# vsois/hanabi-agents

Measured on AMD Instinct MI355X. Metric: env_steps_per_sec, higher is better.
Workload: dtype u8 env/encoder + bfloat16 Q-net GEMM (fp32 accumulate, fp32 master weights)

## Files before the change

### hanabi-agents_amd/csrc/actor_fused.hip

```cpp
#include <hip/hip_runtime.h>
#include <hip/hip_bf16.h>
#include <hip/hip_fp16.h>

#include <cstdint>
#include <type_traits>

#include "../../include/hanabi_hip.h"
#include "common.hpp"
#include "env_kernel.hpp"

using hb::fail;

namespace {

typedef __bf16 bf16x8 __attribute__((ext_vector_type(8)));
typedef _Float16 f16x8 __attribute__((ext_vector_type(8)));
typedef float f32x4 __attribute__((ext_vector_type(4)));

constexpr int FM = 128;
constexpr int FH = 512;
constexpr int FNT = 512;
constexpr int FK = 51;
constexpr int S2 = FH / 32;
constexpr int LUT_BYTES = 65536;
constexpr int H_BYTES = FM * FH * 2;
constexpr int FRAG_FLOATS = 3 * 8 * FM;
constexpr int LDS_TOTAL = H_BYTES + FRAG_FLOATS * 4;
constexpr float NEG_BIG = -1e30f;

struct FusedArgs {
  const uint32_t* obs;
  long long m;
  int words;
  int s1;
  const uint4* w1f;
  const float* b1;
  const uint4* w2f;
  const float* b2;
  const float* support;
  float* q;
  int n_actions, n_pass;
  const int8_t* legal;
  int32_t* actions;
  float epsilon;
  unsigned long long seed, draw;
  long long first_gid;
  unsigned long long* stamps;
};

#ifdef HB_STAMPS
#define HB_FSTAMP(slot)                                                                              \
  do {                                                                                               \
    __builtin_amdgcn_sched_barrier(0);                                                               \
    unsigned long long hb_t_;                                                                        \
    asm volatile("s_memtime %0\n\ts_waitcnt lgkmcnt(0)" : "=s"(hb_t_)::"memory");                    \
    if (a.stamps && lane == 0) a.stamps[(static_cast<long long>(blockIdx.x) * 8 + wave) * 16 + (slot)] = hb_t_; \
    __builtin_amdgcn_sched_barrier(0);                                                               \
  } while (0)
#define HB_FSTAMP_REAL(slot)                                                                         \
  do {                                                                                               \
    unsigned long long hb_t_;                                                                        \
    asm volatile("s_memrealtime %0\n\ts_waitcnt lgkmcnt(0)" : "=s"(hb_t_)::"memory");                \
    if (a.stamps && lane == 0) a.stamps[(static_cast<long long>(blockIdx.x) * 8 + wave) * 16 + (slot)] = hb_t_; \
  } while (0)
#else
#define HB_FSTAMP(slot) do {} while (0)
#define HB_FSTAMP_REAL(slot) do {} while (0)
#endif

template <bool F16>
__device__ __forceinline__ uint32_t pack16(float lo, float hi) {
  if constexpr (F16) {
    const _Float16 a = static_cast<_Float16>(lo), b = static_cast<_Float16>(hi);
    uint16_t ua, ub;
    __builtin_memcpy(&ua, &a, 2);
    __builtin_memcpy(&ub, &b, 2);
    return static_cast<uint32_t>(ua) | (static_cast<uint32_t>(ub) << 16);
  } else {
    const __hip_bfloat16 a = __float2bfloat16(lo), b = __float2bfloat16(hi);
    return static_cast<uint32_t>(*reinterpret_cast<const uint16_t*>(&a)) |
           (static_cast<uint32_t>(*reinterpret_cast<const uint16_t*>(&b)) << 16);
  }
}
template <bool F16>
__device__ __forceinline__ uint32_t bits2_one(uint32_t b, int p) {
  const uint32_t t = (b >> (2 * p)) & 3u;
  return __umul24((t | (t << 15)) & 0x00010001u, F16 ? 0x3C00u : 0x3F80u);
}
template <bool F16>
__device__ __forceinline__ f32x4 mfma16(const uint4& wv, const uint4& xv, const f32x4& c) {
  if constexpr (F16) {
    union { uint4 u; f16x8 f; } w, x;
    w.u = wv; x.u = xv;
    return __builtin_amdgcn_mfma_f32_16x16x32_f16(w.f, x.f, c, 0, 0, 0);
  } else {
    union { uint4 u; bf16x8 f; } w, x;
    w.u = wv; x.u = xv;
    return __builtin_amdgcn_mfma_f32_16x16x32_bf16(w.f, x.f, c, 0, 0, 0);
  }
}
typedef float f32x2 __attribute__((ext_vector_type(2)));
typedef unsigned int u32x2 __attribute__((ext_vector_type(2)));
__device__ __forceinline__ float vmax(float a, float b) {
  float r;
  asm("v_max_f32 %0, %1, %2" : "=v"(r) : "v"(a), "v"(b));
  return r;
}
__device__ __forceinline__ float vmax3(float a, float b, float c) {
  float r;
  asm("v_max3_f32 %0, %1, %2, %3" : "=v"(r) : "v"(a), "v"(b), "v"(c));
  return r;
}
__device__ __forceinline__ float exp2_fast(float x) { return __builtin_amdgcn_exp2f(x); }

template <bool F16, class K, int EG>
__device__ __forceinline__ void actor_fused_body(const FusedArgs& a) {
  __shared__ __attribute__((aligned(16))) unsigned char lds[LDS_TOTAL];
  const int tid = threadIdx.x, lane = tid & 63;
  const int wave = __builtin_amdgcn_readfirstlane(tid >> 6);
  const int r = lane & 15, qd = lane >> 4;
  const long long row0 = static_cast<long long>(blockIdx.x) * FM;
  const int s1 = a.s1, G = (s1 + 3) >> 2;
  unsigned char* lutb = lds + (LDS_TOTAL - LUT_BYTES);
  const int bits_off = LDS_TOTAL - LUT_BYTES - 2048 * G;
  unsigned char* bits = lds + bits_off;
  const int m_early = bits_off >> 14;

  HB_FSTAMP_REAL(14);
  HB_FSTAMP(0);
  const uint4* w1p = a.w1f + (4 * wave) * 64 + lane;
  uint4 wa[4], wb[4];
#pragma unroll
  for (int n = 0; n < 4; ++n) wa[n] = w1p[n * 64];

  uint32_t w[4] = {0u, 0u, 0u, 0u};
  auto load_item = [&](int it) {
    const int rr = it & (FM - 1), g = it >> 7;
    long long row = row0 + rr;
    if (row >= a.m) row = a.m - 1;
    const uint32_t* src = a.obs + row * a.words + 4 * g;
#pragma unroll
    for (int i = 0; i < 4; ++i) w[i] = (4 * g + i < a.words) ? src[i] : 0u;
  };
  if (tid < FM * G) load_item(tid);
  for (int e = tid; e < 4096; e += FNT) {
    const uint32_t v = static_cast<uint32_t>(e) >> 4;
    *reinterpret_cast<uint4*>(lutb + e * 16) = make_uint4(bits2_one<F16>(v, 0), bits2_one<F16>(v, 1), bits2_one<F16>(v, 2), bits2_one<F16>(v, 3));
  }
  for (int it = tid; it < FM * G; it += FNT) {
    const int rr = it & (FM - 1), g = it >> 7;
    if (it != tid) load_item(it);
    uint32_t* dst = reinterpret_cast<uint32_t*>(bits) + (static_cast<size_t>((rr >> 4) * G + g) * 64 + (rr & 15));
#pragma unroll
    for (int qq = 0; qq < 4; ++qq) {
      const uint32_t o = ((w[0] >> (8 * qq)) & 0xFFu) | (((w[1] >> (8 * qq)) & 0xFFu) << 8) | (((w[2] >> (8 * qq)) & 0xFFu) << 16) |
                         (((w[3] >> (8 * qq)) & 0xFFu) << 24);
      dst[qq * 16] = o;
    }
  }
  HB_FSTAMP(1);
  __syncthreads();
  HB_FSTAMP(2);

  f32x4 acc[4][8];
#pragma unroll
  for (int n = 0; n < 4; ++n) {
    const float4 b = *reinterpret_cast<const float4*>(a.b1 + 64 * wave + 16 * n + 4 * qd);
#pragma unroll
    for (int m = 0; m < 8; ++m) acc[n][m] = f32x4{b.x, b.y, b.z, b.w};
  }

  {
    const unsigned char* lut = lutb + r * 16;
    const uint32_t* bw = reinterpret_cast<const uint32_t*>(bits) + lane;
#define HB_L1_STEP(I, WCUR, WNXT, HAVE_NEXT)                                                                   \
  {                                                                                                            \
    const int s_ = 4 * g + (I);                                                                                \
    if (HAVE_NEXT) {                                                                                           \
      _Pragma("unroll") for (int n = 0; n < 4; ++n) WNXT[n] = w1p[(s_ + 1) * 2048 + n * 64];                    \
    }                                                                                                          \
    asm volatile("" ::: "memory");                \
    uint4 xf[8];                                                                                               \
    _Pragma("unroll") for (int m = 0; m < 8; ++m) {                                                            \
      const uint32_t v = (xw[m] >> (8 * (I))) & 0xFFu;                                                         \
      xf[m] = *reinterpret_cast<const uint4*>(lut + v * 256u);                                                 \
    }                                                                                                          \
    _Pragma("unroll") for (int n = 0; n < 4; ++n) {                                                            \
      _Pragma("unroll") for (int m = 0; m < 8; ++m)                                                            \
        acc[n][m] = mfma16<F16>(WCUR[n], xf[m], acc[n][m]);                                                    \
    }                                                                                                          \
  }
    for (int g = 0; g < G; ++g) {
      uint32_t xw[8];
#pragma unroll
      for (int m = 0; m < 8; ++m) xw[m] = bw[(m * G + g) * 64];
      HB_L1_STEP(0, wa, wb, true)
      const bool more = 4 * g + 2 < s1;
      HB_L1_STEP(1, wb, wa, more)
      if (more) {
        HB_L1_STEP(2, wa, wb, true)
        HB_L1_STEP(3, wb, wa, (4 * g + 4 < s1))
      }
    }
#undef HB_L1_STEP
  }
  HB_FSTAMP(3);

  const uint4* w2p = a.w2f + (4 * wave) * 64 + lane;
#pragma unroll
  for (int n = 0; n < 4; ++n) wa[n] = w2p[n * 64];

#define HB_H_WRITE(COND)                                                                                        \
  _Pragma("unroll") for (int m = 0; m < 8; ++m) {                                                               \
    if (COND) {                                                                                                 \
      _Pragma("unroll") for (int n = 0; n < 4; ++n) {                                                           \
        const int chunk = 8 * wave + 2 * n + (qd >> 1);                                                         \
        const float v0 = fmaxf(acc[n][m][0], 0.f), v1 = fmaxf(acc[n][m][1], 0.f);                               \
        const float v2 = fmaxf(acc[n][m][2], 0.f), v3 = fmaxf(acc[n][m][3], 0.f);                               \
        *reinterpret_cast<uint2*>(lds + (16 * m + r) * 1024 + ((chunk ^ r) << 4) + (qd & 1) * 8) =              \
            make_uint2(pack16<F16>(v0, v1), pack16<F16>(v2, v3));                                               \
      }                                                                                                         \
    }                                                                                                           \
  }
  HB_H_WRITE(m < m_early)
  HB_FSTAMP(4);
  __syncthreads();
  HB_H_WRITE(m >= m_early)
#undef HB_H_WRITE

  HB_FSTAMP(5);
  __syncthreads();
  HB_FSTAMP(6);

  const int n_pass = a.n_pass, A = a.n_actions;
  const int full_cap = 8 * n_pass;
  constexpr float LOG2E = 1.44269504088896340736f;
  const unsigned char* hrow = lds + r * 1024;

  for (int p = 0; p < n_pass; ++p) {
    const int slot = 8 * p + wave;
    {
      const float* bp = a.b2 + static_cast<long long>(slot) * 64 + 4 * qd;
#pragma unroll
      for (int n = 0; n < 4; ++n) {
        const float4 b = *reinterpret_cast<const float4*>(bp + 16 * n);
#pragma unroll
        for (int m = 0; m < 8; ++m) acc[n][m] = f32x4{b.x, b.y, b.z, b.w};
      }
    }
    const uint4* wp = w2p + static_cast<long long>(p) * S2 * 2048;
#define HB_L2_HALF(S, WCUR, M0)                                                                                \
  {                                                                                                            \
    uint4 xf[4];                                                                                               \
    const int ch = ((4 * (S) + qd) ^ r) << 4;                                                                  \
    _Pragma("unroll") for (int m = 0; m < 4; ++m) xf[m] = *reinterpret_cast<const uint4*>(hrow + ((M0) + m) * 16384 + ch); \
    _Pragma("unroll") for (int n = 0; n < 4; ++n) {                                                            \
      _Pragma("unroll") for (int m = 0; m < 4; ++m)                                                            \
        acc[n][(M0) + m] = mfma16<F16>(WCUR[n], xf[m], acc[n][(M0) + m]);                                      \
    }                                                                                                          \
  }
#define HB_L2_STEP(S, WCUR, WNXT, HAVE_NEXT)                                                                   \
  {                                                                                                            \
    if (HAVE_NEXT) {                                                                                           \
      _Pragma("unroll") for (int n = 0; n < 4; ++n) WNXT[n] = wp[((S) + 1) * 2048 + n * 64];                    \
    }                                                                                                          \
    asm volatile("" ::: "memory");                                                                             \
    HB_L2_HALF(S, WCUR, 0)                                                                                     \
    __builtin_amdgcn_sched_barrier(0);                                                                         \
    HB_L2_HALF(S, WCUR, 4)                                                                                     \
  }
#pragma unroll 1
    for (int s = 0; s < S2; s += 2) {
      HB_L2_STEP(s, wa, wb, true)
      HB_L2_STEP(s + 1, wb, wa, (s + 2 < S2))
    }
#undef HB_L2_STEP
#undef HB_L2_HALF
    if (p < 2) HB_FSTAMP(7 + 3 * p);
    if (p + 1 < n_pass) {
#pragma unroll
      for (int n = 0; n < 4; ++n) wa[n] = wp[S2 * 2048 + n * 64];
    }

    auto sup_at = [&](int k) { return a.support[k < FK ? k : FK - 1]; };
    f32x2 supF[6];
#pragma unroll
    for (int i = 0; i < 6; ++i) supF[i] = f32x2{sup_at(4 * (2 * i) + qd), sup_at(4 * (2 * i + 1) + qd)};
    const float supF12 = sup_at(48 + qd);
    const int fq = wave & 3;
    const f32x2 supZa = f32x2{sup_at(13 * fq + qd), sup_at(13 * fq + 4 + qd)};
    const f32x2 supZb = f32x2{sup_at(13 * fq + 8 + qd), sup_at(13 * fq + 12)};
    const bool full_ok = slot < A && slot < full_cap;
    float* fb = reinterpret_cast<float*>(lds + H_BYTES) + wave * FM;
    const f32x2 L2 = f32x2{LOG2E, LOG2E};
    hb::static_for<2>([&](auto MH) {
    constexpr int M0 = 4 * decltype(MH)::value;
    float qF[4], zm[4], zs[4], zt[4], vf12[4], vz3[4], nmx[4], nmz[4];
#define HB_M for (int m = 0; m < 4; ++m)
#define HB_SWAP16(X, OP) { const u32x2 t_ = __builtin_amdgcn_permlane16_swap(__float_as_uint(X), __float_as_uint(X), false, false); \
                           X = OP(__uint_as_float(t_.x), __uint_as_float(t_.y)); }
#define HB_SWAP32(X, OP) { const u32x2 t_ = __builtin_amdgcn_permlane32_swap(__float_as_uint(X), __float_as_uint(X), false, false); \
                           X = OP(__uint_as_float(t_.x), __uint_as_float(t_.y)); }
#define HB_ADD(A_, B_) ((A_) + (B_))
#pragma unroll
    HB_M { vf12[m] = qd < 3 ? acc[3][M0 + m][0] : NEG_BIG; vz3[m] = qd == 3 ? acc[3][M0 + m][0] : NEG_BIG; }
#pragma unroll
    HB_M nmx[m] = vmax3(acc[0][M0 + m][0], acc[0][M0 + m][1], acc[0][M0 + m][2]);
#pragma unroll
    HB_M nmx[m] = vmax3(nmx[m], acc[0][M0 + m][3], acc[1][M0 + m][0]);
#pragma unroll
    HB_M nmx[m] = vmax3(nmx[m], acc[1][M0 + m][1], acc[1][M0 + m][2]);
#pragma unroll
    HB_M nmx[m] = vmax3(nmx[m], acc[1][M0 + m][3], acc[2][M0 + m][0]);
#pragma unroll
    HB_M nmx[m] = vmax3(nmx[m], acc[2][M0 + m][1], acc[2][M0 + m][2]);
#pragma unroll
    HB_M nmx[m] = vmax3(nmx[m], acc[2][M0 + m][3], vf12[m]);
#pragma unroll
    HB_M nmz[m] = vmax(vmax3(acc[3][M0 + m][1], acc[3][M0 + m][2], acc[3][M0 + m][3]), vz3[m]);
#pragma unroll
    HB_M HB_SWAP16(nmx[m], vmax)
#pragma unroll
    HB_M HB_SWAP16(nmz[m], vmax)
#pragma unroll
    HB_M HB_SWAP32(nmx[m], vmax)
#pragma unroll
    HB_M HB_SWAP32(nmz[m], vmax)
#pragma unroll
    HB_M { nmx[m] *= -LOG2E; nmz[m] *= -LOG2E; }
    f32x2 s2[4], t2[4];
#define HB_PAIR_FIRST(N, LO, SUP)                                                                   \
  _Pragma("unroll") HB_M {                                                                          \
    const f32x2 arg = f32x2{acc[N][M0 + m][LO], acc[N][M0 + m][LO + 1]} * L2 + f32x2{nmx[m], nmx[m]};         \
    const f32x2 e = f32x2{exp2_fast(arg.x), exp2_fast(arg.y)};                                      \
    s2[m] = e;                                                                                      \
    t2[m] = e * SUP;                                                                                \
  }
#define HB_PAIR(N, LO, SUP)                                                                         \
  _Pragma("unroll") HB_M {                                                                          \
    const f32x2 arg = f32x2{acc[N][M0 + m][LO], acc[N][M0 + m][LO + 1]} * L2 + f32x2{nmx[m], nmx[m]};         \
    const f32x2 e = f32x2{exp2_fast(arg.x), exp2_fast(arg.y)};                                      \
    s2[m] += e;                                                                                     \
    t2[m] += e * SUP;                                                                               \
  }
    HB_PAIR_FIRST(0, 0, supF[0])
    HB_PAIR(0, 2, supF[1])
    HB_PAIR(1, 0, supF[2])
    HB_PAIR(1, 2, supF[3])
    HB_PAIR(2, 0, supF[4])
    HB_PAIR(2, 2, supF[5])
#undef HB_PAIR
#undef HB_PAIR_FIRST
    float sF[4], tF[4];
#pragma unroll
    HB_M {
      const float e12 = exp2_fast(vf12[m] * LOG2E + nmx[m]);
      sF[m] = s2[m].x + s2[m].y + e12;
      tF[m] = t2[m].x + t2[m].y + e12 * supF12;
    }
#pragma unroll
    HB_M {
      const f32x2 arg = f32x2{acc[3][M0 + m][1], acc[3][M0 + m][2]} * L2 + f32x2{nmz[m], nmz[m]};
      const f32x2 e = f32x2{exp2_fast(arg.x), exp2_fast(arg.y)};
      s2[m] = e;
      t2[m] = e * supZa;
    }
#pragma unroll
    HB_M {
      const f32x2 arg = f32x2{acc[3][M0 + m][3], vz3[m]} * L2 + f32x2{nmz[m], nmz[m]};
      const f32x2 e = f32x2{exp2_fast(arg.x), exp2_fast(arg.y)};
      s2[m] += e;
      t2[m] += e * supZb;
    }
#pragma unroll
    HB_M { zs[m] = s2[m].x + s2[m].y; zt[m] = t2[m].x + t2[m].y; }
#pragma unroll
    HB_M HB_SWAP16(sF[m], HB_ADD)
#pragma unroll
    HB_M HB_SWAP16(tF[m], HB_ADD)
#pragma unroll
    HB_M HB_SWAP16(zs[m], HB_ADD)
#pragma unroll
    HB_M HB_SWAP16(zt[m], HB_ADD)
#pragma unroll
    HB_M HB_SWAP32(sF[m], HB_ADD)
#pragma unroll
    HB_M HB_SWAP32(tF[m], HB_ADD)
#pragma unroll
    HB_M HB_SWAP32(zs[m], HB_ADD)
#pragma unroll
    HB_M HB_SWAP32(zt[m], HB_ADD)
#pragma unroll
    HB_M { zm[m] = -nmz[m]; qF[m] = tF[m] * __builtin_amdgcn_rcpf(sF[m]) * (1.0f / FK); }
#undef HB_M
#undef HB_SWAP16
#undef HB_SWAP32
#undef HB_ADD
    if (qd == 0) {
#pragma unroll
      for (int m = 0; m < 4; ++m) {
        const long long row = row0 + 16 * (M0 + m) + r;
        if (full_ok && row < a.m) a.q[row * A + slot] = qF[m];
        fb[16 * (M0 + m) + r] = zm[m];
        fb[8 * FM + 16 * (M0 + m) + r] = zs[m];
        fb[16 * FM + 16 * (M0 + m) + r] = zt[m];
      }
    }
    __builtin_amdgcn_sched_barrier(0);
    });
    if (p < 2) HB_FSTAMP(8 + 3 * p);
    __syncthreads();
    if (tid < 2 * FM) {
      const int rr = tid & (FM - 1), g = tid >> 7;
      const int ea = full_cap + 2 * p + g;
      const long long row = row0 + rr;
      if (ea < A && row < a.m) {
        const float* f = reinterpret_cast<const float*>(lds + H_BYTES) + (4 * g) * FM + rr;
        const float m0 = f[0], m1 = f[FM], m2 = f[2 * FM], m3 = f[3 * FM];
        const float M = fmaxf(fmaxf(m0, m1), fmaxf(m2, m3));
        const float e0 = exp2_fast(m0 - M), e1 = exp2_fast(m1 - M), e2 = exp2_fast(m2 - M), e3 = exp2_fast(m3 - M);
        const float* fs = f + 8 * FM;
        const float* ft = f + 16 * FM;
        const float S = fs[0] * e0 + fs[FM] * e1 + fs[2 * FM] * e2 + fs[3 * FM] * e3;
        const float T = ft[0] * e0 + ft[FM] * e1 + ft[2 * FM] * e2 + ft[3 * FM] * e3;
        a.q[row * A + ea] = T * __builtin_amdgcn_rcpf(S) * (1.0f / FK);
      }
    }
    if (p + 1 < n_pass) __syncthreads();
    if (p < 2) HB_FSTAMP(9 + 3 * p);
  }
  if (a.legal) {
    asm volatile("s_waitcnt vmcnt(0)" ::: "memory");
    __syncthreads();
    if (tid < FM && row0 + tid < a.m) {
      const long long g = row0 + tid;
      const unsigned long long gid = static_cast<unsigned long long>(a.first_gid + g);
      uint32_t rnd[4];
      hb::philox4x32_10(static_cast<uint32_t>(a.draw), static_cast<uint32_t>(a.draw >> 32), static_cast<uint32_t>(gid),
                        static_cast<uint32_t>(gid >> 32), static_cast<uint32_t>(a.seed), static_cast<uint32_t>(a.seed >> 32), rnd);
      const float* qr = a.q + g * A;
      const int8_t* lr = a.legal + g * A;
      float best = -INFINITY;
      unsigned long long legal_mask = 0, ties = 0;
      for (int i = 0; i < A; ++i) {
        const float v = __hip_atomic_load(qr + i, __ATOMIC_RELAXED, __HIP_MEMORY_SCOPE_AGENT);
        if (lr[i] != 0) {
          legal_mask |= 1ull << i;
          if (v > best) { best = v; ties = 1ull << i; }
          else if (v == best) ties |= 1ull << i;
        }
      }
      const float u = static_cast<float>(rnd[0] >> 8) * (1.0f / 16777216.0f);
      unsigned long long pool = (u < a.epsilon) ? legal_mask : ties;
      if (pool == 0) pool = legal_mask;
      int pick = 0;
      const int c = __popcll(pool);
      if (c > 0) {
        int k = static_cast<int>(__umulhi(rnd[1], static_cast<uint32_t>(c)));
        while (k-- > 0) pool &= pool - 1;
        pick = __ffsll(static_cast<long long>(pool)) - 1;
      }
      a.actions[g] = pick;
      if constexpr (!std::is_void_v<K>) reinterpret_cast<int*>(lds + H_BYTES)[tid] = pick;
    }
  }
  if constexpr (!std::is_void_v<K>) {
    constexpr int ENV_WORDS = hb::env_lds_words<K, EG>();
    static_assert((FM / EG) * ENV_WORDS * 4 <= H_BYTES && FM / EG <= FNT / 64, "env tail: the LDS slices must fit in H");
    __syncthreads();
    if (wave < FM / EG) {
#if defined(__HIP_DEVICE_COMPILE__)
      typedef const __attribute__((address_space(4))) unsigned char KargByte;
      typedef const __attribute__((address_space(4))) hb::EnvArgs KargEnv;
      auto kargs = __builtin_amdgcn_kernarg_segment_ptr();
      asm volatile("" : "+s"(kargs));
      constexpr size_t ENV_OFF = (sizeof(FusedArgs) + alignof(hb::EnvArgs) - 1) / alignof(hb::EnvArgs) * alignof(hb::EnvArgs);
      KargEnv& env = *(KargEnv*)((KargByte*)kargs + ENV_OFF);
#else
      const hb::EnvArgs env{};
#endif
      const long long g0 = row0 + EG * wave;
      const int uid = lane < EG ? reinterpret_cast<const int*>(lds + H_BYTES)[EG * wave + lane] : 0;
      hb::env_wave_step<K, EG>(env, g0, lane, reinterpret_cast<uint32_t*>(lds) + wave * ENV_WORDS, uid, g0 / EG);
    }
  }
  HB_FSTAMP_REAL(15);
}

template <bool F16>
__global__ __launch_bounds__(FNT) void actor_fused_kernel(const FusedArgs a) {
  actor_fused_body<F16, void, 16>(a);
}

template <bool F16, class K, int EG>
__global__ __launch_bounds__(FNT) void actor_env_fused_kernel(const FusedArgs a, const hb::EnvArgs env) {
  (void)env;
  actor_fused_body<F16, K, EG>(a);
}

template <bool F16>
__global__ __launch_bounds__(FNT) void actor_fused_grouped_kernel(const FusedArgs a, const hb_fused_tile* __restrict__ tiles) {
  const hb_fused_tile& t = tiles[blockIdx.x];
  if (!t.active) return;
  FusedArgs b = a;
  b.w1f = static_cast<const uint4*>(t.w1f); b.b1 = t.b1f; b.w2f = static_cast<const uint4*>(t.w2f); b.b2 = t.b2f;
  b.support = t.support;
  b.first_gid = t.first_game_id - static_cast<long long>(blockIdx.x) * FM;
  actor_fused_body<F16, void, 16>(b);
}

struct PackArgs {
  const __hip_bfloat16* w1; int w1_ld;
  const __hip_bfloat16* b1;
  const __hip_bfloat16* w2; int w2_ld;
  const __hip_bfloat16* b2;
  int obs_len, s1, n_actions, n_pass;
  uint4* w1f; float* b1f; uint4* w2f; float* b2f;
  int chunks1, chunks2;
  int f16;
  uint16_t* w1t; int w1t_ld;
  uint16_t* w2t; int w2t_ld;
};
__device__ __forceinline__ float bias_to_float(const __hip_bfloat16* b, int i, int f16) {
  return f16 ? __half2float(reinterpret_cast<const __half*>(b)[i]) : __bfloat162float(b[i]);
}
__host__ __device__ __forceinline__ int fused_logit(int col, int n_actions, int n_pass) {
  const int slot = col >> 6, c = col & 63, n = c >> 4, q = (c >> 2) & 3, j = c & 3;
  const int r16 = 4 * n + j;
  const int full_cap = 8 * n_pass;
  int action, atom;
  if (r16 < 12 || (r16 == 12 && q < 3)) {
    action = slot < full_cap ? slot : n_actions;
    if (action >= n_actions) return -1;
    atom = r16 < 12 ? 4 * r16 + q : 48 + q;
  } else {
    const int p = slot >> 3, w = slot & 7, f = w & 3;
    action = full_cap + 2 * p + (w >> 2);
    atom = r16 == 12 ? 13 * f + 12 : 13 * f + 4 * (r16 - 13) + q;
  }
  if (action >= n_actions || atom >= FK) return -1;
  return action * FK + atom;
}
__global__ __launch_bounds__(256) void actor_fused_pack_kernel(const PackArgs a) {
  const int id = static_cast<int>(blockIdx.x) * 256 + static_cast<int>(threadIdx.x);
  const __hip_bfloat16 zero = __float2bfloat16(0.f);
  if (id < a.chunks1) {
    const int lane = id & 63, nt = (id >> 6) & 31, s = id >> 11;
    const int unit = 16 * nt + (lane & 15), k0 = 32 * s + 8 * (lane >> 4);
    __hip_bfloat16 v[8];
#pragma unroll
    for (int i = 0; i < 8; ++i) v[i] = (k0 + i < a.obs_len) ? a.w1[static_cast<long long>(k0 + i) * a.w1_ld + unit] : zero;
    a.w1f[id] = *reinterpret_cast<const uint4*>(v);
    if (a.w1t) *reinterpret_cast<uint4*>(a.w1t + static_cast<size_t>(unit) * a.w1t_ld + k0) = *reinterpret_cast<const uint4*>(v);
    if (id < FH) a.b1f[id] = bias_to_float(a.b1, id, a.f16);
  } else if (id < a.chunks1 + a.chunks2) {
    const int id2 = id - a.chunks1;
    const int lane = id2 & 63, ntp = (id2 >> 6) & 31, s = (id2 >> 11) % S2, pass = (id2 >> 11) / S2;
    const int col = 16 * (32 * pass + ntp) + (lane & 15), k0 = 32 * s + 8 * (lane >> 4);
    const int lg = fused_logit(col, a.n_actions, a.n_pass);
    __hip_bfloat16 v[8];
#pragma unroll
    for (int i = 0; i < 8; ++i) v[i] = lg >= 0 ? a.w2[static_cast<long long>(k0 + i) * a.w2_ld + lg] : zero;
    a.w2f[id2] = *reinterpret_cast<const uint4*>(v);
    if (a.w2t && lg >= 0) *reinterpret_cast<uint4*>(a.w2t + static_cast<size_t>(lg) * a.w2t_ld + k0) = *reinterpret_cast<const uint4*>(v);
    if (s == 0 && (lane >> 4) == 0) a.b2f[col] = lg >= 0 ? bias_to_float(a.b2, lg, a.f16) : NEG_BIG;
  }
}

// ... 113 lines not shown
                       int64_t first_game_id, int32_t* actions_dev, void* stream) {
  return hb_actor_fused_act_dt(obs_bits_dev, legal_dev, n_rows, obs_len, w1f_dev, b1f_dev, w2f_dev, b2f_dev, support_dev, hidden,
                               n_actions, n_atoms, q_dev, epsilon, seed, draw, first_game_id, actions_dev, 1, stream);
}

int hb_actor_fused_act_grouped(const hb_fused_tile* tiles_dev, int64_t n_rows, const uint32_t* obs_bits_dev, const int8_t* legal_dev,
                               int32_t obs_len, int32_t hidden, int32_t n_actions, int32_t n_atoms, float* q_dev, float epsilon,
                               uint64_t seed, uint64_t draw, int32_t* actions_dev, int32_t dtype, void* stream) {
  if (dtype != 1 && dtype != 2) return fail(HB_ERR_INVALID, "dtype must be 1 (bf16) or 2 (f16)");
  if (!tiles_dev || !obs_bits_dev || !legal_dev || !q_dev || !actions_dev) return fail(HB_ERR_INVALID, "null argument");
  if (!hb_actor_fused_supported(obs_len, hidden, n_actions, n_atoms)) return fail(HB_ERR_INVALID, "shape not covered by the fused actor kernel");
  if (n_actions > 64) return fail(HB_ERR_INVALID, "n_actions must be 1..64 for the fused selection");
  if (n_rows < 0 || n_rows % FM) return fail(HB_ERR_INVALID, "n_rows (%lld) must be a multiple of %d: one tile descriptor per %d rows",
                                             static_cast<long long>(n_rows), FM, FM);
  if (n_rows / FM > 0x7fffffff) return fail(HB_ERR_INVALID, "too many tiles");
  if (n_rows == 0) return HB_OK;
  FusedArgs a{};
  a.obs = obs_bits_dev; a.m = n_rows; a.words = (obs_len + 31) / 32; a.s1 = 2 * ((obs_len + 63) / 64);
  a.q = q_dev; a.n_actions = n_actions; a.n_pass = passes_for(n_actions);
  a.legal = legal_dev; a.actions = actions_dev; a.epsilon = epsilon; a.seed = seed; a.draw = draw;
  const dim3 grid(static_cast<unsigned>(n_rows / FM));
  if (dtype == 2) hipLaunchKernelGGL(actor_fused_grouped_kernel<true>, grid, dim3(FNT), 0, static_cast<hipStream_t>(stream), a, tiles_dev);
  else hipLaunchKernelGGL(actor_fused_grouped_kernel<false>, grid, dim3(FNT), 0, static_cast<hipStream_t>(stream), a, tiles_dev);
  HB_HIP(hipGetLastError());
  return HB_OK;
}

#ifdef HB_STAMPS
int hb_actor_fused_q_stamped(const uint32_t* obs_bits_dev, int64_t n_rows, int32_t obs_len, const void* w1f_dev, const float* b1f_dev,
                             const void* w2f_dev, const float* b2f_dev, const float* support_dev, int32_t hidden, int32_t n_actions,
                             int32_t n_atoms, float* q_dev, unsigned long long* stamps_dev, void* stream) {
  return fused_launch(obs_bits_dev, n_rows, obs_len, w1f_dev, b1f_dev, w2f_dev, b2f_dev, support_dev, hidden, n_actions, n_atoms, q_dev,
                      stamps_dev, nullptr, 1, stream);
}
#endif

static int fused_args(const uint32_t* obs_bits_dev, int64_t n_rows, int32_t obs_len, const void* w1f_dev, const float* b1f_dev,
                      const void* w2f_dev, const float* b2f_dev, const float* support_dev, int32_t hidden, int32_t n_actions,
                      int32_t n_atoms, float* q_dev, unsigned long long* stamps_dev, const FusedSelect* sel, int32_t dtype, FusedArgs& a,
                      bool* launch) {
  *launch = false;
  if (dtype != 1 && dtype != 2) return fail(HB_ERR_INVALID, "dtype must be 1 (bf16) or 2 (f16)");
  if (!obs_bits_dev || !w1f_dev || !b1f_dev || !w2f_dev || !b2f_dev || !support_dev || !q_dev) return fail(HB_ERR_INVALID, "null argument");
  if (!hb_actor_fused_supported(obs_len, hidden, n_actions, n_atoms)) return fail(HB_ERR_INVALID, "shape not covered by the fused actor kernel");
  if (n_rows <= 0) return HB_OK;
  if (!aligned16(w1f_dev) || !aligned16(w2f_dev) || !aligned16(b1f_dev) || !aligned16(b2f_dev))
    return fail(HB_ERR_ALIGN, "w1f / w2f / b1f / b2f must be 16-byte aligned");
  a = FusedArgs{};
  a.obs = obs_bits_dev; a.m = n_rows; a.words = (obs_len + 31) / 32; a.s1 = 2 * ((obs_len + 63) / 64);
  a.w1f = static_cast<const uint4*>(w1f_dev); a.b1 = b1f_dev; a.w2f = static_cast<const uint4*>(w2f_dev); a.b2 = b2f_dev;
  a.support = support_dev; a.q = q_dev; a.n_actions = n_actions; a.n_pass = passes_for(n_actions);
  a.stamps = stamps_dev;
  if (sel) {
    a.legal = sel->legal; a.actions = sel->actions; a.epsilon = sel->epsilon; a.seed = sel->seed; a.draw = sel->draw;
    a.first_gid = sel->first_gid;
  }
  *launch = true;
  return HB_OK;
}

static int fused_launch(const uint32_t* obs_bits_dev, int64_t n_rows, int32_t obs_len, const void* w1f_dev, const float* b1f_dev,
                        const void* w2f_dev, const float* b2f_dev, const float* support_dev, int32_t hidden, int32_t n_actions,
                        int32_t n_atoms, float* q_dev, unsigned long long* stamps_dev, const FusedSelect* sel, int32_t dtype, void* stream) {
  FusedArgs a;
  bool go = false;
  if (int rc = fused_args(obs_bits_dev, n_rows, obs_len, w1f_dev, b1f_dev, w2f_dev, b2f_dev, support_dev, hidden, n_actions, n_atoms, q_dev,
                          stamps_dev, sel, dtype, a, &go))
    return rc;
  if (!go) return HB_OK;
  const dim3 grid(static_cast<unsigned>((n_rows + FM - 1) / FM));
  if (dtype == 2) hipLaunchKernelGGL(actor_fused_kernel<true>, grid, dim3(FNT), 0, static_cast<hipStream_t>(stream), a);
  else hipLaunchKernelGGL(actor_fused_kernel<false>, grid, dim3(FNT), 0, static_cast<hipStream_t>(stream), a);
  HB_HIP(hipGetLastError());
  return HB_OK;
}

}

namespace {

using ActEnvFull2 = hb::Cfg<2, 5, 5, 5, 8, 3>;
using ActEnvFull5 = hb::Cfg<5, 5, 5, 4, 8, 3>;
constexpr int ENV_EG = 16;

template <class K>
static bool is_cfg(const hb::EnvVariant& v) {
  return v.P == K::P && v.C == K::C && v.R == K::R && v.H == K::H && v.INFO == K::INFO && v.LIFE == K::LIFE;
}

template <bool F16, class K>
static void launch_act_env(const FusedArgs& a, const hb::EnvArgs& env, dim3 grid, hipStream_t stream) {
  if (env.ev_start && env.ev_stop)
    hipExtLaunchKernelGGL((actor_env_fused_kernel<F16, K, ENV_EG>), grid, dim3(FNT), 0, stream, env.ev_start, env.ev_stop, 0, a, env);
  else
    hipLaunchKernelGGL((actor_env_fused_kernel<F16, K, ENV_EG>), grid, dim3(FNT), 0, stream, a, env);
}

}

namespace hb {

bool actor_env_fused_supported(const EnvVariant& v) { return is_cfg<ActEnvFull2>(v) || is_cfg<ActEnvFull5>(v); }

int actor_env_fused_launch(const uint32_t* obs_bits_dev, const int8_t* legal_dev, int64_t n_rows, int32_t obs_len, const void* w1f_dev,
                           const float* b1f_dev, const void* w2f_dev, const float* b2f_dev, const float* support_dev, int32_t hidden,
                           int32_t n_actions, int32_t n_atoms, float* q_dev, float epsilon, uint64_t seed, uint64_t draw,
                           int64_t first_game_id, int32_t* actions_dev, int32_t dtype, const EnvArgs& env, const EnvVariant& var,
                           void* stream) {
  if (!legal_dev || !actions_dev) return fail(HB_ERR_INVALID, "null argument");
  if (!actor_env_fused_supported(var)) return fail(HB_ERR_INVALID, "no fused policy + env kernel for this game configuration");
  if (n_rows != env.n) return fail(HB_ERR_INVALID, "n_rows (%lld) must equal the env's game count (%lld)", static_cast<long long>(n_rows), env.n);
  if (n_actions != var.n_actions || obs_len != var.obs_len) return fail(HB_ERR_INVALID, "actor shape does not match the env");
  const FusedSelect sel{legal_dev, actions_dev, epsilon, seed, draw, first_game_id};
  FusedArgs a;
  bool go = false;
  if (int rc = fused_args(obs_bits_dev, n_rows, obs_len, w1f_dev, b1f_dev, w2f_dev, b2f_dev, support_dev, hidden, n_actions, n_atoms, q_dev,
                          nullptr, &sel, dtype, a, &go))
    return rc;
  if (!go) return HB_OK;
  const dim3 grid(static_cast<unsigned>((n_rows + FM - 1) / FM));
  const hipStream_t st = static_cast<hipStream_t>(stream);
  const bool f16 = dtype == 2;
  if (is_cfg<ActEnvFull2>(var)) {
    if (f16) launch_act_env<true, ActEnvFull2>(a, env, grid, st);
    else launch_act_env<false, ActEnvFull2>(a, env, grid, st);
  } else {
    if (f16) launch_act_env<true, ActEnvFull5>(a, env, grid, st);
    else launch_act_env<false, ActEnvFull5>(a, env, grid, st);
  }
  HB_HIP(hipGetLastError());
  return HB_OK;
}

}
```

### hanabi-agents_amd/csrc/env_kernel.hpp

```cpp
#pragma once
#include <hip/hip_runtime.h>
#include <hip/hip_ext.h>
#include <stdint.h>
#include <utility>

namespace hb {

enum { MODE_STEP = 0, MODE_OBSERVE = 1, MODE_RESET = 2 };
constexpr int NEXT_DECK_BYTES = 64;
enum { MV_PLAY = 0, MV_DISCARD = 1, MV_RCOLOR = 2, MV_RRANK = 3 };

struct EnvArgs {
  uint32_t* state;
  const int32_t* actions;
  const uint8_t* mask;
  const uint8_t* decks;
  uint8_t* next_deck;
  uint8_t* refill;
  int8_t* obs;
  uint32_t* obs_bits;
  int8_t* legal;
  float* reward;
  int8_t* terminal;
  float* agent_reward;
// ... 211 lines not shown
      }
#pragma unroll
      for (int u = 0; u < 4; ++u) {
        if (c0 + 64 * u < chunks) {
          u32x4 o;
          o.x = spread4(v[u]);
          o.y = spread4(v[u] >> 4);
          o.z = spread4(v[u] >> 8);
          o.w = spread4(v[u] >> 12);
          __builtin_nontemporal_store(o, reinterpret_cast<u32x4_unaligned*>(out + off[u]));
        }
      }
    }
  }
  if constexpr (TAIL > 0) {
    const int n = nvalid * TAIL;
    for (int e = lane; e < n; e += 64) {
      const int g = e / TAIL, j = e - g * TAIL, k = CPR * 16 + j;
      out[g * L + k] = static_cast<int8_t>((bits[g * row_stride + (k >> 5)] >> (k & 31)) & 1u);
    }
  }
}

template <int A>
__device__ __forceinline__ int select_action(const EnvArgs& a, long long gi) {
  float qv[A];
  uint32_t lw[(A + 3) / 4];
  const float* qr = a.sel_q + gi * A;
  const int8_t* lr = a.sel_legal + gi * A;
  if constexpr (A % 4 == 0) {
#pragma unroll
    for (int i = 0; i < A / 4; ++i) {
      const float4 v = reinterpret_cast<const float4*>(qr)[i];
      qv[4 * i] = v.x; qv[4 * i + 1] = v.y; qv[4 * i + 2] = v.z; qv[4 * i + 3] = v.w;
      lw[i] = reinterpret_cast<const uint32_t*>(lr)[i];
    }
  } else {
#pragma unroll
    for (int i = 0; i < (A + 3) / 4; ++i) lw[i] = 0;
#pragma unroll
    for (int i = 0; i < A; ++i) {
      qv[i] = qr[i];
      lw[i >> 2] |= static_cast<uint32_t>(static_cast<uint8_t>(lr[i])) << (8 * (i & 3));
    }
  }
  const unsigned long long gid = static_cast<unsigned long long>(a.sel_first_gid + gi);
  uint32_t r[4];
  philox4x32_10(static_cast<uint32_t>(a.sel_draw), static_cast<uint32_t>(a.sel_draw >> 32), static_cast<uint32_t>(gid),
                static_cast<uint32_t>(gid >> 32), static_cast<uint32_t>(a.sel_seed), static_cast<uint32_t>(a.sel_seed >> 32), r);
  float best = -INFINITY;
  unsigned long long legal_mask = 0, ties = 0;
#pragma unroll
  for (int i = 0; i < A; ++i) {
    const float v = qv[i];
    if ((lw[i >> 2] >> (8 * (i & 3))) & 0xFFu) {
      legal_mask |= 1ull << i;
      if (v > best) { best = v; ties = 1ull << i; }
      else if (v == best) ties |= 1ull << i;
    }
  }
  const float u = static_cast<float>(r[0] >> 8) * (1.0f / 16777216.0f);
  unsigned long long pool = (u < a.sel_eps) ? legal_mask : ties;
  if (pool == 0) pool = legal_mask;
  int pick = 0;
  const int c = __popcll(pool);
  if (c > 0) {
    int k = static_cast<int>(__umulhi(r[1], static_cast<uint32_t>(c)));
    while (k-- > 0) pool &= pool - 1;
    pick = __ffsll(static_cast<long long>(pool)) - 1;
  }
  a.sel_actions[gi] = pick;
  return pick;
}

__device__ __forceinline__ void wave_sync() {
  __builtin_amdgcn_fence(__ATOMIC_RELEASE, "wavefront");
  __builtin_amdgcn_wave_barrier();
  __builtin_amdgcn_fence(__ATOMIC_ACQUIRE, "wavefront");
}

template <class K, int G>
constexpr int env_lds_words() { return G * (K::SWP + K::NWP + K::LW); }

template <class K, int G, bool SHUF = false>
__device__ __forceinline__ void env_wave_step(const EnvArgs& a, long long g0, int lane, uint32_t* const srow, int uid_in,
                                              long long wslot) {
  constexpr int P = K::P, C = K::C, R = K::R, H = K::H;
  constexpr int LPG = 1;
  uint32_t* const obits = srow + G * K::SWP;
  uint32_t* const lbits = obits + G * K::NWP;
  const long long left = a.n - g0;
  const int nvalid = left <= 0 ? 0 : (left < G ? static_cast<int>(left) : G);
  const int mode = a.mode;
  HB_STAMP_REAL(10);
  HB_STAMP(0);

  const bool active = lane < nvalid && lane < G;
  const long long gi = g0 + lane;
  bool mask_in = true;
  uint4 nd[4] = {make_uint4(0u, 0u, 0u, 0u), make_uint4(0u, 0u, 0u, 0u), make_uint4(0u, 0u, 0u, 0u), make_uint4(0u, 0u, 0u, 0u)};
  const uint4* const ndp = reinterpret_cast<const uint4*>(a.next_deck + gi * NEXT_DECK_BYTES);
  if (active) {
    if (mode == MODE_RESET && a.mask) mask_in = a.mask[gi] != 0;
    if (mode == MODE_RESET && mask_in) {
      nd[0] = ndp[0]; nd[1] = ndp[1]; nd[2] = ndp[2]; nd[3] = ndp[3];
    }
  }
  uint4 pm = make_uint4(0u, 0u, 0u, 0u);
  if constexpr (SHUF) {
    if (active) pm = reinterpret_cast<const uint4*>(a.perms)[gi];
  }

  {
    constexpr int Q = K::SW / 4;
    constexpr int ROUNDS = (G * Q + 63) / 64;
    const uint4* src = reinterpret_cast<const uint4*>(a.state + g0 * K::SW);
    uint4 v[ROUNDS];
#pragma unroll
    for (int r = 0; r < ROUNDS; ++r) {
      const int e = lane + 64 * r;
      v[r] = e < nvalid * Q ? src[e] : make_uint4(0u, 0u, 0u, 0u);
    }
#pragma unroll
    for (int r = 0; r < ROUNDS; ++r) {
      const int e = lane + 64 * r;
      if (e < nvalid * Q) {
        const int g = e / Q, q = e - g * Q;
        uint32_t* d = srow + g * K::SWP + 4 * q;
        d[0] = v[r].x; d[1] = v[r].y; d[2] = v[r].z; d[3] = v[r].w;
      }
    }
  }
  HB_STAMP(1);
  wave_sync();
  HB_STAMP(2);

  uint32_t* const row = srow + lane * K::SWP;
  uint32_t w0 = 0, w1 = 0, w2 = 0, w3 = 0, w6 = 0;
  uint64_t accw = 0, disc = 0;
  float out_reward = 0.f;
  int out_term = 0, out_score = 0;
  bool illegal = false, need_reset = false, keep_seats = true;
  int reset_start = 0;

  auto hand_n = [&](int p) -> int { return (w1 >> (15 + 3 * p)) & 7; };
  auto fw = [&](int c) -> int { return (w1 >> (3 * c)) & 7; };
  auto score_now = [&]() -> int {
    if (((w0 >> 10) & 7) == 0) return 0;
    int s = 0;
#pragma unroll
    for (int c = 0; c < C; ++c) s += fw(c);
    return s;
  };

  if (active) {
    w0 = row[0]; w1 = row[1]; w2 = row[2]; w3 = row[3]; w6 = row[6];
    accw = (static_cast<uint64_t>(row[5]) << 32) | row[4];
    disc = (static_cast<uint64_t>(row[9]) << 32) | row[8];
    if (mode == MODE_RESET) {
      need_reset = mask_in;
      keep_seats = false;
      reset_start = a.start_player;
    } else if (mode == MODE_STEP && ((w0 >> 19) & 3) == 0) {
      {
        int fsum = 0;
#pragma unroll
        for (int c = 0; c < C; ++c) fsum += fw(c);
        if (((w0 >> 10) & 7) <= 1 || (w0 & 63) == 0 || fsum >= C * R - 1) {
          nd[0] = ndp[0]; nd[1] = ndp[1]; nd[2] = ndp[2]; nd[3] = ndp[3];
        }
      }
      if constexpr (SHUF) {
        const int xc0 = uid_in - 2 * H;
        if (xc0 >= 0 && xc0 < (P - 1) * C) {
          const uint32_t sgm = perm_of(pm, (w0 >> 13) & 7);
          const int tgt = xc0 / C, seen = xc0 - tgt * C;
          int c = 0;
#pragma unroll
          for (int k = 0; k < C; ++k) c = static_cast<int>((sgm >> (3 * k)) & 7u) == seen ? k : c;
          uid_in = 2 * H + tgt * C + c;
        }
      }
      const int deck_size = w0 & 63, info = (w0 >> 6) & 15, life = (w0 >> 10) & 7;
      const int s = (w0 >> 13) & 7;
      const int turns = (w0 >> 16) & 7, moves = (w0 >> 21) & 255;
      const bool in_range = uid_in >= 0 && uid_in < K::A;
      const int uid = in_range ? uid_in : 0;
      const bool is_discard = uid < H, is_play = uid >= H && uid < 2 * H;
      const bool is_rc = uid >= 2 * H && uid < 2 * H + (P - 1) * C, is_rr = uid >= 2 * H + (P - 1) * C;
      const bool card_move = is_discard || is_play, is_hint = !card_move;
      const int type = is_play ? MV_PLAY : (is_discard ? MV_DISCARD : (is_rc ? MV_RCOLOR : MV_RRANK));
      const int xc = uid - 2 * H, xr = uid - 2 * H - (P - 1) * C;
      const int ci = is_discard ? uid : (is_play ? uid - H : 0);
      const int toff = is_rc ? 1 + xc / C : (is_rr ? 1 + xr / R : 0);
      const int hcol = is_rc ? xc % C : 0, hrank = is_rr ? xr % R : 0;
      int t = s + toff;
// ... 455 lines not shown
```

Baseline: 313.1 million.

## Overlap env-state loads with the final Q pass and distribute action selection per wave

In the fused actor+env kernel, the last pass's merge of extra actions and its q values are written to an LDS tile, and the final global round-trip is skipped. Action selection moves from threads 0..127 into the per-wave env tail: each wave's lanes select for their own games and feed the pick straight into env_wave_step. Legal masks, earlier-pass q values, Philox draws and the env state rows are issued before the final barrier, so their global latency overlaps the end of the GEMM. This adds register pressure and couples the LDS layout tightly, guarded by static asserts. A 4-byte alignment check on legal is added, and stamp slots widen for profiling.

Result: slower. 309.0 million (-1.3%).

```diff
diff --git a/hanabi-agents_amd/csrc/actor_fused.hip b/hanabi-agents_amd/csrc/actor_fused.hip
--- a/hanabi-agents_amd/csrc/actor_fused.hip
+++ b/hanabi-agents_amd/csrc/actor_fused.hip
@@ -48,20 +48,21 @@
   unsigned long long* stamps;
 };
 
+#define HB_FSTAMP_SLOTS 32
 #ifdef HB_STAMPS
 #define HB_FSTAMP(slot)                                                                              \
   do {                                                                                               \
     __builtin_amdgcn_sched_barrier(0);                                                               \
     unsigned long long hb_t_;                                                                        \
     asm volatile("s_memtime %0\n\ts_waitcnt lgkmcnt(0)" : "=s"(hb_t_)::"memory");                    \
-    if (a.stamps && lane == 0) a.stamps[(static_cast<long long>(blockIdx.x) * 8 + wave) * 16 + (slot)] = hb_t_; \
+    if (a.stamps && lane == 0) a.stamps[(static_cast<long long>(blockIdx.x) * 8 + wave) * HB_FSTAMP_SLOTS + (slot)] = hb_t_; \
     __builtin_amdgcn_sched_barrier(0);                                                               \
   } while (0)
 #define HB_FSTAMP_REAL(slot)                                                                         \
   do {                                                                                               \
     unsigned long long hb_t_;                                                                        \
     asm volatile("s_memrealtime %0\n\ts_waitcnt lgkmcnt(0)" : "=s"(hb_t_)::"memory");                \
-    if (a.stamps && lane == 0) a.stamps[(static_cast<long long>(blockIdx.x) * 8 + wave) * 16 + (slot)] = hb_t_; \
+    if (a.stamps && lane == 0) a.stamps[(static_cast<long long>(blockIdx.x) * 8 + wave) * HB_FSTAMP_SLOTS + (slot)] = hb_t_; \
   } while (0)
 #else
 #define HB_FSTAMP(slot) do {} while (0)
@@ -116,6 +117,7 @@
 template <bool F16, class K, int EG>
 __device__ __forceinline__ void actor_fused_body(const FusedArgs& a) {
   __shared__ __attribute__((aligned(16))) unsigned char lds[LDS_TOTAL];
+  constexpr bool TAIL = !std::is_void_v<K>;
   const int tid = threadIdx.x, lane = tid & 63;
   const int wave = __builtin_amdgcn_readfirstlane(tid >> 6);
   const int r = lane & 15, qd = lane >> 4;
@@ -237,6 +239,29 @@
   constexpr float LOG2E = 1.44269504088896340736f;
   const unsigned char* hrow = lds + r * 1024;
 
+  auto merge_extras = [&](int tid, int p, float* qt) {
+    if (tid < 2 * FM) {
+      const int rr = tid & (FM - 1), g = tid >> 7;
+      const int ea = full_cap + 2 * p + g;
+      const long long row = row0 + rr;
+      if (ea < A && row < a.m) {
+#pragma clang fp contract(off)
+        const float* f = reinterpret_cast<const float*>(lds + H_BYTES) + (4 * g) * FM + rr;
+        const float m0 = f[0], m1 = f[FM], m2 = f[2 * FM], m3 = f[3 * FM];
+        const float M = fmaxf(fmaxf(m0, m1), fmaxf(m2, m3));
+        const float e0 = exp2_fast(m0 - M), e1 = exp2_fast(m1 - M), e2 = exp2_fast(m2 - M), e3 = exp2_fast(m3 - M);
+        const float* fs = f + 8 * FM;
+        const float* ft = f + 16 * FM;
+        const float S = fs[0] * e0 + fs[FM] * e1 + fs[2 * FM] * e2 + fs[3 * FM] * e3;
+        const float T = ft[0] * e0 + ft[FM] * e1 + ft[2 * FM] * e2 + ft[3 * FM] * e3;
+        const float qe = T * __builtin_amdgcn_rcpf(S) * (1.0f / FK);
+        a.q[row * A + ea] = qe;
+        if (qt) qt[ea * FM + rr] = qe;
+      }
+    }
+  };
+  float qlast0 = 0.f, qlast1 = 0.f;
+
   for (int p = 0; p < n_pass; ++p) {
     const int slot = 8 * p + wave;
     {
@@ -277,6 +302,10 @@
 #undef HB_L2_STEP
 #undef HB_L2_HALF
     if (p < 2) HB_FSTAMP(7 + 3 * p);
+    if (p + 1 == n_pass) HB_FSTAMP(16);
+    if constexpr (TAIL) {
+      if (p + 1 == n_pass && p > 0) asm volatile("s_waitcnt vmcnt(0)" ::: "memory");
+    }
     if (p + 1 < n_pass) {
 #pragma unroll
       for (int n = 0; n < 4; ++n) wa[n] = wp[S2 * 2048 + n * 64];
@@ -406,32 +435,112 @@
         fb[16 * FM + 16 * (M0 + m) + r] = zt[m];
       }
     }
+    if constexpr (TAIL) {
+      const float k0 = (qd & 1) ? qF[2] : qF[0], k1 = (qd & 1) ? qF[3] : qF[1];
+      if constexpr (M0 == 0) { qlast0 = k0; qlast1 = k1; }
+      else { qlast0 = qd >= 2 ? k0 : qlast0; qlast1 = qd >= 2 ? k1 : qlast1; }
+    }
     __builtin_amdgcn_sched_barrier(0);
     });
     if (p < 2) HB_FSTAMP(8 + 3 * p);
+    if (p + 1 == n_pass) HB_FSTAMP(17);
     __syncthreads();
-    if (tid < 2 * FM) {
-      const int rr = tid & (FM - 1), g = tid >> 7;
-      const int ea = full_cap + 2 * p + g;
-      const long long row = row0 + rr;
-      if (ea < A && row < a.m) {
-        const float* f = reinterpret_cast<const float*>(lds + H_BYTES) + (4 * g) * FM + rr;
-        const float m0 = f[0], m1 = f[FM], m2 = f[2 * FM], m3 = f[3 * FM];
-        const float M = fmaxf(fmaxf(m0, m1), fmaxf(m2, m3));
-        const float e0 = exp2_fast(m0 - M), e1 = exp2_fast(m1 - M), e2 = exp2_fast(m2 - M), e3 = exp2_fast(m3 - M);
-        const float* fs = f + 8 * FM;
-        const float* ft = f + 16 * FM;
-        const float S = fs[0] * e0 + fs[FM] * e1 + fs[2 * FM] * e2 + fs[3 * FM] * e3;
-        const float T = ft[0] * e0 + ft[FM] * e1 + ft[2 * FM] * e2 + ft[3 * FM] * e3;
-        a.q[row * A + ea] = T * __builtin_amdgcn_rcpf(S) * (1.0f / FK);
-      }
-    }
+    if constexpr (TAIL) {
+      if (p + 1 == n_pass) break;
+    }
+    merge_extras(tid, p, nullptr);
     if (p + 1 < n_pass) __syncthreads();
     if (p < 2) HB_FSTAMP(9 + 3 * p);
-  }
-  if (a.legal) {
+    if (p + 1 == n_pass) HB_FSTAMP(18);
+  }
+  if constexpr (TAIL) {
+    constexpr int TA = K::A, TNP = (TA + 9) / 10, TCAP = 8 * TNP, PL = TNP - 1;
+    constexpr int ENV_WORDS = hb::env_lds_words<K, EG>();
+    constexpr int QT_OFF = ((FM / EG) * ENV_WORDS * 4 + 15) / 16 * 16;
+    static_assert(QT_OFF + TA * FM * 4 <= H_BYTES && FM / EG == FNT / 64 && TA % 4 == 0,
+                  "env tail: the env slices and the q tile must fit in H; one wavefront per EG games");
+    float* const qt = reinterpret_cast<float*>(lds + QT_OFF);
+    constexpr auto pass_of = [](int i) constexpr { return i < TCAP ? i / 8 : (i - TCAP) / 2; };
+#if defined(__HIP_DEVICE_COMPILE__)
+    typedef const __attribute__((address_space(4))) unsigned char KargByte;
+    typedef const __attribute__((address_space(4))) hb::EnvArgs KargEnv;
+    auto kargs = __builtin_amdgcn_kernarg_segment_ptr();
+    asm volatile("" : "+s"(kargs));
+    constexpr size_t ENV_OFF = (sizeof(FusedArgs) + alignof(hb::EnvArgs) - 1) / alignof(hb::EnvArgs) * alignof(hb::EnvArgs);
+    KargEnv& env = *(KargEnv*)((KargByte*)kargs + ENV_OFF);
+#else
+    const hb::EnvArgs env{};
+#endif
+    const int lane = static_cast<int>(__builtin_amdgcn_mbcnt_hi(~0u, __builtin_amdgcn_mbcnt_lo(~0u, 0u)));
+    const int tid = 64 * wave + lane, r = lane & 15, qd = lane >> 4;
+    const long long g0 = row0 + EG * wave, gsel = g0 + lane;
+    const bool sel = lane < EG && gsel < a.m;
+    uint32_t lw[TA / 4];
+    float qv[TA];
+    if (sel) {
+      const uint32_t* lr = reinterpret_cast<const uint32_t*>(a.legal + gsel * TA);
+#pragma unroll
+      for (int i = 0; i < TA / 4; ++i) lw[i] = lr[i];
+#pragma unroll
+      for (int i = 0; i < TA; ++i)
+        if (pass_of(i) < PL) qv[i] = __hip_atomic_load(a.q + gsel * TA + i, __ATOMIC_RELAXED, __HIP_MEMORY_SCOPE_AGENT);
+    }
+    hb::EnvRows<K, EG> rows;
+    const int nvalid = hb::env_nvalid<K, EG>(a.m, g0);
+    hb::env_rows_request<K, EG>(env.state, g0, nvalid, lane, rows);
+    uint32_t rnd[4] = {0u, 0u, 0u, 0u};
+    if (sel) {
+      const unsigned long long gid = static_cast<unsigned long long>(a.first_gid + gsel);
+      hb::philox4x32_10(static_cast<uint32_t>(a.draw), static_cast<uint32_t>(a.draw >> 32), static_cast<uint32_t>(gid),
+                        static_cast<uint32_t>(gid >> 32), static_cast<uint32_t>(a.seed), static_cast<uint32_t>(a.seed >> 32), rnd);
+    }
+    merge_extras(tid, PL, qt);
+    {
+      const int slot = 8 * PL + wave;
+      if (slot < TA) {
+        qt[slot * FM + 32 * qd + r] = qlast0;
+        qt[slot * FM + 32 * qd + 16 + r] = qlast1;
+      }
+    }
+    HB_FSTAMP(18);
+    HB_FSTAMP(19);
+    __syncthreads();
+    HB_FSTAMP(20);
+    int pick = 0;
+    if (sel) {
+#pragma unroll
+      for (int i = 0; i < TA; ++i)
+        if (pass_of(i) == PL) qv[i] = qt[i * FM + EG * wave + lane];
+      float best = -INFINITY;
+      unsigned long long legal_mask = 0, ties = 0;
+#pragma unroll
+      for (int i = 0; i < TA; ++i) {
+        const float v = qv[i];
+        if ((lw[i >> 2] >> (8 * (i & 3))) & 0xFFu) {
+          legal_mask |= 1ull << i;
+          if (v > best) { best = v; ties = 1ull << i; }
+          else if (v == best) ties |= 1ull << i;
+        }
+      }
+      const float u = static_cast<float>(rnd[0] >> 8) * (1.0f / 16777216.0f);
+      unsigned long long pool = (u < a.epsilon) ? legal_mask : ties;
+      if (pool == 0) pool = legal_mask;
+      const int c = __popcll(pool);
+      if (c > 0) {
+        int k = static_cast<int>(__umulhi(rnd[1], static_cast<uint32_t>(c)));
+        while (k-- > 0) pool &= pool - 1;
+        pick = __ffsll(static_cast<long long>(pool)) - 1;
+      }
+      a.actions[gsel] = pick;
+    }
+    HB_FSTAMP(21);
+    HB_FSTAMP(22);
+    hb::env_wave_step<K, EG, false, true>(env, g0, lane, reinterpret_cast<uint32_t*>(lds) + wave * ENV_WORDS, pick, g0 / EG, &rows);
+  } else if (a.legal) {
     asm volatile("s_waitcnt vmcnt(0)" ::: "memory");
+    HB_FSTAMP(19);
     __syncthreads();
+    HB_FSTAMP(20);
     if (tid < FM && row0 + tid < a.m) {
       const long long g = row0 + tid;
       const unsigned long long gid = static_cast<unsigned long long>(a.first_gid + g);
@@ -461,29 +570,10 @@
         pick = __ffsll(static_cast<long long>(pool)) - 1;
       }
       a.actions[g] = pick;
-      if constexpr (!std::is_void_v<K>) reinterpret_cast<int*>(lds + H_BYTES)[tid] = pick;
-    }
-  }
-  if constexpr (!std::is_void_v<K>) {
-    constexpr int ENV_WORDS = hb::env_lds_words<K, EG>();
-    static_assert((FM / EG) * ENV_WORDS * 4 <= H_BYTES && FM / EG <= FNT / 64, "env tail: the LDS slices must fit in H");
-    __syncthreads();
-    if (wave < FM / EG) {
-#if defined(__HIP_DEVICE_COMPILE__)
-      typedef const __attribute__((address_space(4))) unsigned char KargByte;
-      typedef const __attribute__((address_space(4))) hb::EnvArgs KargEnv;
-      auto kargs = __builtin_amdgcn_kernarg_segment_ptr();
-      asm volatile("" : "+s"(kargs));
-      constexpr size_t ENV_OFF = (sizeof(FusedArgs) + alignof(hb::EnvArgs) - 1) / alignof(hb::EnvArgs) * alignof(hb::EnvArgs);
-      KargEnv& env = *(KargEnv*)((KargByte*)kargs + ENV_OFF);
-#else
-      const hb::EnvArgs env{};
-#endif
-      const long long g0 = row0 + EG * wave;
-      const int uid = lane < EG ? reinterpret_cast<const int*>(lds + H_BYTES)[EG * wave + lane] : 0;
-      hb::env_wave_step<K, EG>(env, g0, lane, reinterpret_cast<uint32_t*>(lds) + wave * ENV_WORDS, uid, g0 / EG);
-    }
-  }
+    }
+    HB_FSTAMP(21);
+  }
+  HB_FSTAMP(23);
   HB_FSTAMP_REAL(15);
 }
 
@@ -763,6 +853,10 @@
 using ActEnvFull2 = hb::Cfg<2, 5, 5, 5, 8, 3>;
 using ActEnvFull5 = hb::Cfg<5, 5, 5, 4, 8, 3>;
 constexpr int ENV_EG = 16;
+#ifdef HB_STAMPS
+unsigned long long* g_tail_stamps = nullptr;
+unsigned long long* g_tail_env_stamps = nullptr;
+#endif
 
 template <class K>
 static bool is_cfg(const hb::EnvVariant& v) {
@@ -778,6 +872,14 @@
 }
 
 }
+
+#ifdef HB_STAMPS
+extern "C" int hb_actor_fused_tail_stamps(unsigned long long* fused_stamps_dev, unsigned long long* env_stamps_dev) {
+  g_tail_stamps = fused_stamps_dev;
+  g_tail_env_stamps = env_stamps_dev;
+  return HB_OK;
+}
+#endif
 
 namespace hb {
 
@@ -792,6 +894,7 @@
   if (!actor_env_fused_supported(var)) return fail(HB_ERR_INVALID, "no fused policy + env kernel for this game configuration");
   if (n_rows != env.n) return fail(HB_ERR_INVALID, "n_rows (%lld) must equal the env's game count (%lld)", static_cast<long long>(n_rows), env.n);
   if (n_actions != var.n_actions || obs_len != var.obs_len) return fail(HB_ERR_INVALID, "actor shape does not match the env");
+  if (reinterpret_cast<uintptr_t>(legal_dev) & 3) return fail(HB_ERR_ALIGN, "legal_dev must be 4-byte aligned");
   const FusedSelect sel{legal_dev, actions_dev, epsilon, seed, draw, first_game_id};
   FusedArgs a;
   bool go = false;
@@ -802,12 +905,20 @@
   const dim3 grid(static_cast<unsigned>((n_rows + FM - 1) / FM));
   const hipStream_t st = static_cast<hipStream_t>(stream);
   const bool f16 = dtype == 2;
+#ifdef HB_STAMPS
+  EnvArgs env_stamped = env;
+  env_stamped.stamps = g_tail_env_stamps;
+  a.stamps = g_tail_stamps;
+  const EnvArgs& envk = env_stamped;
+#else
+  const EnvArgs& envk = env;
+#endif
   if (is_cfg<ActEnvFull2>(var)) {
-    if (f16) launch_act_env<true, ActEnvFull2>(a, env, grid, st);
-    else launch_act_env<false, ActEnvFull2>(a, env, grid, st);
+    if (f16) launch_act_env<true, ActEnvFull2>(a, envk, grid, st);
+    else launch_act_env<false, ActEnvFull2>(a, envk, grid, st);
   } else {
-    if (f16) launch_act_env<true, ActEnvFull5>(a, env, grid, st);
-    else launch_act_env<false, ActEnvFull5>(a, env, grid, st);
+    if (f16) launch_act_env<true, ActEnvFull5>(a, envk, grid, st);
+    else launch_act_env<false, ActEnvFull5>(a, envk, grid, st);
   }
   HB_HIP(hipGetLastError());
   return HB_OK;
diff --git a/hanabi-agents_amd/csrc/env_kernel.hpp b/hanabi-agents_amd/csrc/env_kernel.hpp
--- a/hanabi-agents_amd/csrc/env_kernel.hpp
+++ b/hanabi-agents_amd/csrc/env_kernel.hpp
@@ -317,9 +317,44 @@
 template <class K, int G>
 constexpr int env_lds_words() { return G * (K::SWP + K::NWP + K::LW); }
 
-template <class K, int G, bool SHUF = false>
+template <class K, int G>
+struct EnvRows {
+  static constexpr int Q = K::SW / 4;
+  static constexpr int ROUNDS = (G * Q + 63) / 64;
+  uint4 v[ROUNDS];
+};
+template <class K, int G>
+__device__ __forceinline__ int env_nvalid(long long n, long long g0) {
+  const long long left = n - g0;
+  return left <= 0 ? 0 : (left < G ? static_cast<int>(left) : G);
+}
+template <class K, int G>
+__device__ __forceinline__ void env_rows_request(const uint32_t* state, long long g0, int nvalid, int lane, EnvRows<K, G>& rows) {
+  constexpr int Q = EnvRows<K, G>::Q;
+  const uint4* src = reinterpret_cast<const uint4*>(state + g0 * K::SW);
+#pragma unroll
+  for (int r = 0; r < EnvRows<K, G>::ROUNDS; ++r) {
+    const int e = lane + 64 * r;
+    rows.v[r] = e < nvalid * Q ? src[e] : make_uint4(0u, 0u, 0u, 0u);
+  }
+}
+template <class K, int G>
+__device__ __forceinline__ void env_rows_place(const EnvRows<K, G>& rows, int nvalid, int lane, uint32_t* const srow) {
+  constexpr int Q = EnvRows<K, G>::Q;
+#pragma unroll
+  for (int r = 0; r < EnvRows<K, G>::ROUNDS; ++r) {
+    const int e = lane + 64 * r;
+    if (e < nvalid * Q) {
+      const int g = e / Q, q = e - g * Q;
+      uint32_t* d = srow + g * K::SWP + 4 * q;
+      d[0] = rows.v[r].x; d[1] = rows.v[r].y; d[2] = rows.v[r].z; d[3] = rows.v[r].w;
+    }
+  }
+}
+
+template <class K, int G, bool SHUF = false, bool PRE = false>
 __device__ __forceinline__ void env_wave_step(const EnvArgs& a, long long g0, int lane, uint32_t* const srow, int uid_in,
-                                              long long wslot) {
+                                              long long wslot, const EnvRows<K, G>* rows = nullptr) {
   constexpr int P = K::P, C = K::C, R = K::R, H = K::H;
   constexpr int LPG = 1;
   uint32_t* const obits = srow + G * K::SWP;
@@ -346,7 +381,9 @@
     if (active) pm = reinterpret_cast<const uint4*>(a.perms)[gi];
   }
 
-  {
+  if constexpr (PRE) {
+    env_rows_place<K, G>(*rows, nvalid, lane, srow);
+  } else {
     constexpr int Q = K::SW / 4;
     constexpr int ROUNDS = (G * Q + 63) / 64;
     const uint4* src = reinterpret_cast<const uint4*>(a.state + g0 * K::SW);
```
